# Lagrange-Labs/mapreduce-plonky2

Hardware: AMD Instinct MI355X
Metric: leaf proofs/sec (whole node) + NTT GB/s vs HBM peak, 2^20-row table build, 1/2/4/8 GPU (higher is better)
Workload: dtype u64 (Goldilocks field)

## Files before the change

include/mp2g.h:

```cpp
#ifndef MP2G_H
#define MP2G_H
#include <stddef.h>
#include <stdint.h>
#ifdef __cplusplus
extern "C" {
#endif

typedef struct mp2g_ctx mp2g_ctx;
typedef struct mp2g_tree mp2g_tree;
typedef struct mp2g_batch mp2g_batch;

#define MP2G_POSEIDON2 0
#define MP2G_POSEIDON 1

uint64_t mp2g_stat_leaf_permutations(void);
const char* mp2g_last_error(void);
int mp2g_device_count(void);
int mp2g_ctx_create(int device, mp2g_ctx** out);
void mp2g_ctx_destroy(mp2g_ctx* ctx);
int mp2g_ctx_sync(mp2g_ctx* ctx);
int mp2g_ctx_make_current(mp2g_ctx* ctx);
int mp2g_ctx_mem_info(mp2g_ctx* ctx, size_t* free_bytes, size_t* total_bytes);
void* mp2g_ctx_stream(mp2g_ctx* ctx);
int mp2g_ctx_set_stream(mp2g_ctx* ctx, void* stream);
// ... 9 lines not shown
int mp2g_timer_stop(mp2g_ctx* ctx, float* ms);

int mp2g_ntt(mp2g_ctx* ctx, uint64_t* data, uint32_t log_n, uint32_t batch, int inverse,
             uint64_t coset_shift, int bitrev_out);
int mp2g_ntt_dev(mp2g_ctx* ctx, const uint64_t* d_in, uint64_t* d_out, uint32_t log_n, uint32_t batch,
                 int inverse, uint64_t coset_shift, int bitrev_out);
int mp2g_lde_leaves(mp2g_ctx* ctx, const uint64_t* coeffs, uint32_t log_n, uint32_t w, uint32_t rate_bits,
                    uint64_t* leaves);
int mp2g_lde_dev(mp2g_ctx* ctx, const uint64_t* d_coeffs, uint32_t log_n, uint32_t w, uint32_t rate_bits,
                 uint64_t* d_values);

int mp2g_hash_no_pad_batch(mp2g_ctx* ctx, int variant, const uint64_t* in, uint32_t in_len, uint32_t count,
                           uint32_t out_len, uint64_t* out);
int mp2g_hash_no_pad_batch_dev(mp2g_ctx* ctx, int variant, const uint64_t* d_in, uint32_t in_len,
                               uint32_t count, uint32_t out_len, uint64_t* d_out);
int mp2g_merkle_build(mp2g_ctx* ctx, int variant, const uint64_t* leaves, uint32_t leaf_len,
                      uint32_t log_leaves, uint32_t cap_height, mp2g_tree** out);
int mp2g_merkle_cap(const mp2g_tree* tree, uint64_t* cap );
int mp2g_merkle_open(const mp2g_tree* tree, const uint32_t* idx, uint32_t n_idx, uint64_t* leaves_out,
                     uint64_t* siblings_out);
void mp2g_merkle_free(mp2g_tree* tree);

int mp2g_commit_from_values(mp2g_ctx* ctx, int variant, const uint64_t* values, uint32_t log_n, uint32_t w,
                            uint32_t rate_bits, uint32_t cap_height, mp2g_batch** out);
int mp2g_commit_from_values_dev(mp2g_ctx* ctx, int variant, const uint64_t* d_values, uint32_t log_n,
                                uint32_t w, uint32_t rate_bits, uint32_t cap_height, mp2g_batch** out);
int mp2g_commit_from_coeffs_dev(mp2g_ctx* ctx, int variant, const uint64_t* d_coeffs, uint32_t log_n,
                                uint32_t w, uint32_t rate_bits, uint32_t cap_height, mp2g_batch** out);
int mp2g_recommit_from_values_dev(mp2g_ctx* ctx, mp2g_batch* batch, const uint64_t* d_values);
int mp2g_batch_rehash_dev(mp2g_ctx* ctx, mp2g_batch* batch, int parts);
// ... 21 lines not shown
uint32_t mp2g_reduction_arity_bits(uint32_t degree_bits, uint32_t rate_bits, uint32_t cap_height,
                                   uint32_t arity_bits, uint32_t final_poly_bits, uint32_t* out);
size_t mp2g_fri_proof_words(const mp2g_fri_params* p);
size_t mp2g_fri_n_openings(const mp2g_fri_params* p);

typedef struct mp2g_challenger mp2g_challenger;
int mp2g_challenger_create(mp2g_ctx* ctx, int variant, uint32_t count, mp2g_challenger** out);
int mp2g_challenger_observe(mp2g_challenger* ch, const uint64_t* elems, uint32_t n);
int mp2g_challenger_get(mp2g_challenger* ch, uint32_t n, uint64_t* out );
void mp2g_challenger_free(mp2g_challenger* ch);

int mp2g_fri_fold(mp2g_ctx* ctx, const uint64_t* evals, uint32_t log_m, uint32_t arity_bits,
                  const uint64_t beta[2], uint64_t shift, uint64_t* out);
int mp2g_fri_pow(mp2g_ctx* ctx, int variant, const uint64_t state[12], uint32_t pos, uint32_t bits,
                 uint64_t* witness);

int mp2g_batch_eval_ext(const mp2g_batch* batch, const uint64_t point[2], uint64_t* out );
int mp2g_fri_prove(mp2g_ctx* ctx, const mp2g_fri_params* params, mp2g_batch* const* oracles, const uint64_t zeta[2],
                   mp2g_challenger* ch, uint64_t* proof);

typedef struct mp2g_prover mp2g_prover;
int mp2g_prover_create(mp2g_ctx* ctx, const mp2g_fri_params* params, uint32_t batch, mp2g_prover** out);
int mp2g_prover_set_preprocessed_dev(mp2g_prover* pr, const uint64_t* d_values);
int mp2g_prover_prove_dev(mp2g_prover* pr, const uint64_t* const* d_values, const uint64_t* d_circuit_digest,
                          const uint64_t* d_pi_hash, uint64_t* d_caps, uint64_t* d_openings, uint64_t* d_proof);
void mp2g_prover_free(mp2g_prover* pr);
int mp2g_pcs_prove(mp2g_ctx* ctx, const mp2g_fri_params* params, const uint64_t* const* values,
                   const uint64_t circuit_digest[4], const uint64_t pi_hash[4], uint64_t* caps,
                   uint64_t* openings, uint64_t* proof);

// ... 236 lines not shown
```

mapreduce-plonky2_amd/__init__.py:

```python
import ctypes
import time
import os
import weakref

import numpy as np

_HERE = os.path.dirname(os.path.abspath(__file__))
LIB_PATH = os.environ.get("MP2G_LIB", os.path.join(_HERE, "libmp2gpu.so"))
HEADER_PATH = os.path.join(os.path.dirname(_HERE), "include", "mp2g.h")

P = 0xFFFFFFFF00000001
MULT_GEN = 14293326489335486720
POSEIDON2, POSEIDON = 0, 1

_u64p = ctypes.POINTER(ctypes.c_uint64)
_u32p = ctypes.POINTER(ctypes.c_uint32)
_lib = None


class Mp2gError(RuntimeError):
    pass


def load():
# ... 161 lines not shown
        _ck(load().mp2g_lde_leaves(self.h, _p(c), log_n, w, rate_bits, _p(out)))
        return out

    def lde_dev(self, d_coeffs, log_n, w, rate_bits, d_values):
        _ck(load().mp2g_lde_dev(self.h, d_coeffs.ptr, log_n, w, rate_bits, d_values.ptr))

    def hash_no_pad_batch(self, inputs, out_len=4, variant=POSEIDON2):
        a = _arr(inputs)
        count, in_len = a.shape
        out = np.empty((count, out_len), dtype=np.uint64)
        _ck(load().mp2g_hash_no_pad_batch(self.h, variant, _p(a), in_len, count, out_len, _p(out)))
        return out

    def hash_no_pad(self, values, variant=POSEIDON2):
        return self.hash_no_pad_batch(_arr(values).reshape(1, -1), 4, variant)[0]


class MerkleTree:

    def __init__(self, ctx, leaves, cap_height, variant=POSEIDON2):
        a = _arr(leaves)
        L, leaf_len = a.shape
        self.log_leaves = int(L).bit_length() - 1
        assert 1 << self.log_leaves == L
        self.ctx, self.cap_height, self.leaf_len = ctx, cap_height, leaf_len
        self.h = ctypes.c_void_p()
        _ck(load().mp2g_merkle_build(ctx.h, variant, _p(a), leaf_len, self.log_leaves, cap_height, ctypes.byref(self.h)))
        ctx._adopt(self)

    @property
# ... 160 lines not shown
def fri_fold(ctx, evals, arity_bits, beta, shift):
    a = _arr(evals)
    m = a.shape[0]
    log_m = int(m).bit_length() - 1
    out = np.empty((m >> arity_bits, 2), dtype=np.uint64)
    b = _arr(beta)
    _ck(load().mp2g_fri_fold(ctx.h, _p(a), log_m, arity_bits, _p(b), ctypes.c_uint64(shift), _p(out)))
    return out


def fri_pow(ctx, state, pos, bits, variant=POSEIDON2):
    s = _arr(state)
    w = ctypes.c_uint64()
    _ck(load().mp2g_fri_pow(ctx.h, variant, _p(s), pos, bits, ctypes.byref(w)))
    return w.value


def pcs_prove(ctx, fp, values, circuit_digest, pi_hash):
    vals = [_arr(v) for v in values]
    ptrs = (ctypes.c_void_p * len(vals))(*[v.ctypes.data for v in vals])
    caps = np.empty((fp.n_oracles, fp.cap_words), dtype=np.uint64)
    openings = np.empty((fp.n_openings, 2), dtype=np.uint64)
    proof = np.empty(fp.proof_words, dtype=np.uint64)
    cd, ph = _arr(circuit_digest), _arr(pi_hash)
    _ck(load().mp2g_pcs_prove(ctx.h, ctypes.byref(fp), ptrs, _p(cd), _p(ph), _p(caps), _p(openings), _p(proof)))
    return caps, openings, proof


class Gate(ctypes.Structure):
    _fields_ = [("kind", ctypes.c_uint32), ("p0", ctypes.c_uint32), ("p1", ctypes.c_uint32), ("p2", ctypes.c_uint32),
# ... 572 lines not shown
```

mapreduce-plonky2_amd/csrc/api.hip:

```cpp
#include "ctx.h"
#include <cstdlib>
#include <cstdarg>
#include <cstdio>
#include <cstring>
#include <new>

using namespace mp2g;

static thread_local char g_err[512] = "";
int mp2g::fail(const char* fmt, ...) {
  va_list ap;
  va_start(ap, fmt);
  vsnprintf(g_err, sizeof g_err, fmt, ap);
  va_end(ap);
  return 1;
}

extern "C" {

const char* mp2g_last_error(void) { return g_err; }

int mp2g_device_count(void) {
  int n = 0;
  if (hipGetDeviceCount(&n) != hipSuccess) return 0;
// ... 195 lines not shown
  NEED(out_len >= 1, "out_len >= 1");
  CK(hash_no_pad_batch(c->stream, variant, (const u64*)d_in, in_len, count, out_len, (u64*)d_out));
  return 0;
}
int mp2g_hash_no_pad_batch(mp2g_ctx* c, int variant, const uint64_t* in, uint32_t in_len, uint32_t count,
                           uint32_t out_len, uint64_t* out) {
  NEED(c && out, "ctx/out");
  if (count == 0) return 0;
  DevBuf di, dout;
  CK(di.alloc((size_t)count * in_len * sizeof(u64)));
  CK(dout.alloc((size_t)count * out_len * sizeof(u64)));
  if (in_len) CK(hipMemcpyAsync(di.p, in, (size_t)count * in_len * sizeof(u64), hipMemcpyHostToDevice, c->stream));
  int rc = mp2g_hash_no_pad_batch_dev(c, variant, di.p, in_len, count, out_len, dout.p);
  if (rc) return rc;
  CK(hipMemcpyAsync(out, dout.p, (size_t)count * out_len * sizeof(u64), hipMemcpyDeviceToHost, c->stream));
  CK(hipStreamSynchronize(c->stream));
  return 0;
}

int mp2g_merkle_build(mp2g_ctx* c, int variant, const uint64_t* leaves, uint32_t leaf_len, uint32_t log_leaves,
                      uint32_t cap_height, mp2g_tree** out) {
  NEED(c && out && (leaves || leaf_len == 0), "ctx/out/leaves");
  NEED(variant == 0 || variant == 1, "variant");
  NEED(log_leaves <= 28, "log_leaves <= 28");
  NEED(cap_height <= log_leaves, "cap_height <= log2(leaves)");
  mp2g_tree* t = new (std::nothrow) mp2g_tree();
  if (!t) return fail("out of memory");
  t->ctx = c; t->variant = variant; t->leaf_len = leaf_len; t->log_leaves = log_leaves; t->cap_h = cap_height;
  const size_t L = (size_t)1 << log_leaves;
  hipError_t e = t->leaves.alloc(L * leaf_len * sizeof(u64));
// ... 176 lines not shown
```

mapreduce-plonky2_amd/csrc/fri.hip:

```cpp
#include "fri.h"
#include "poseidon_wave.cuh"

namespace mp2g {

template <int V>
__device__ void ch_duplex(ChState& c) {
  for (u32 i = 0; i < c.n_in; i++) c.state[i] = c.in[i];
  c.n_in = 0;
  u64 s[12];
#pragma unroll
  for (int i = 0; i < 12; i++) s[i] = c.state[i];
  perm<V>(s);
#pragma unroll
  for (int i = 0; i < 12; i++) c.state[i] = s[i];
#pragma unroll
  for (int i = 0; i < 8; i++) c.out[i] = s[i];
  c.n_out = 8;
}
template <int V>
__global__ void ch_kernel(ChState* st, u32 B, const u64* obs, u64 obs_bstride, u32 n_obs, u64* out, u64 out_bstride, u32 n_get) {
  u32 b = blockIdx.x * blockDim.x + threadIdx.x;
  if (b >= B) return;
  ChState c = st[b];
  const u64* o = obs + b * obs_bstride;
// ... 293 lines not shown
  for (int i = 0; i < 8; i++)
    if ((u32)i < pos) base[i] = c.in[i];
  const u64 stride = (u64)gridDim.x * blockDim.x;
  for (u64 cand = (u64)blockIdx.x * blockDim.x + threadIdx.x;; cand += stride) {
    if (threadIdx.x == 0) s_best = atomicMin(wit, ~0ull);
    __syncthreads();
    const unsigned long long best = s_best;
    __syncthreads();
    if (cand - threadIdx.x > best) break;
    u64 s[12];
#pragma unroll
    for (int i = 0; i < 12; i++) s[i] = base[i];
#pragma unroll
    for (int i = 0; i < 8; i++)
      if ((u32)i == pos) s[i] = cand;
    perm<V>(s);
    if (cand < GL_P && (bits == 0 || (s[7] >> (64 - bits)) == 0)) atomicMin(wit, (unsigned long long)cand);
  }
}
__global__ void fill_u64_kernel(u64* p, u64 v, u32 n) {
  u32 i = blockIdx.x * blockDim.x + threadIdx.x;
  if (i < n) p[i] = v;
}

__global__ void __launch_bounds__(256) query_kernel(FriShape sh, FriLayers ly, FriProofLayout L, const u64* chal ,
                                                      u64 chal_bstride, u64* proof) {
  const u32 q = blockIdx.x, b = blockIdx.y, t = threadIdx.x;
  const u32 lg = L.lg;
  const u64 N = (u64)1 << lg;
  u64 x = chal[b * chal_bstride + q] % N;
  u64* const qs = proof + b * L.proof_words + L.q_off + q * L.q_words;
// ... 105 lines not shown
```

mapreduce-plonky2_amd/csrc/gates.hip:

```cpp
#include "gates.h"
#include "poseidon.cuh"
#include "coset_constants.h"

namespace mp2g {

u32 gate_num_constraints(const mp2g_gate& g) {
  switch (g.kind) {
    case MP2G_GATE_CONSTANT: return g.p0;
    case MP2G_GATE_PUBLIC_INPUT: return 4;
    case MP2G_GATE_ARITHMETIC: return g.p0;
    case MP2G_GATE_BASE_SUM: return 1 + g.p0;
    case MP2G_GATE_ARITHMETIC_EXT: case MP2G_GATE_MUL_EXT: return 2 * g.p0;
    case MP2G_GATE_POSEIDON2: case MP2G_GATE_POSEIDON: return 1 + 4 + 36 + 22 + 48 + 12;
    case MP2G_GATE_POSEIDON_MDS: return 24;
    case MP2G_GATE_COSET_INTERPOLATION: return 4 + 4 * (((1u << g.p0) - 2) / (g.p1 - 1));
    case MP2G_GATE_U32_ARITHMETIC: return 36 * g.p0;
    case MP2G_GATE_U32_RANGE_CHECK: return 17 * g.p0;
    case MP2G_GATE_U32_SUBTRACTION: return 19 * g.p0;
    case MP2G_GATE_U32_ADD_MANY: return 21 * g.p1;
    case MP2G_GATE_COMPARISON: return g.p1 ? 6 + 5 * g.p1 + (g.p0 + g.p1 - 1) / g.p1 : 0;
    case MP2G_GATE_EXPONENTIATION: return g.p0 + 1;
    case MP2G_GATE_REDUCING: case MP2G_GATE_REDUCING_EXT: return 2 * g.p0;
    case MP2G_GATE_RANDOM_ACCESS: return (g.p0 + 2) * g.p1 + g.p2;
    case MP2G_GATE_U32_INTERLEAVE: return 34 * g.p0;
// ... 219 lines not shown
        u64 lhs = wire(i), rhs = wire(i + 4), delta = wire(25 + i);
        emit(gl_sub(gl_mul(swap, gl_sub(rhs, lhs)), delta));
        s[i] = gl_add(lhs, delta);
        s[i + 4] = gl_sub(rhs, delta);
      }
#pragma unroll
      for (int i = 8; i < 12; i++) s[i] = wire(i);
      p2_external(s);
#pragma unroll 1
      for (int r = 0; r < 4; r++) {
        if (r != 0) {
#pragma unroll
          for (int i = 0; i < 12; i++) {
            u64 in = wire(29 + 12 * (r - 1) + i);
            emit(diff(s[i], c_p2_ext[12 * r + i], in));
            s[i] = p2_sbox(in, 0);
          }
        } else {
#pragma unroll
          for (int i = 0; i < 12; i++) s[i] = p2_sbox(s[i], c_p2_ext[i]);
        }
        p2_external(s);
      }
      u64 nxt = wire(65);
#pragma unroll 1
      for (int r = 0; r < 22; r++) {
        const u64 in = nxt;
        if (r < 21) nxt = wire(65 + r + 1);
        emit(diff(s[0], c_p2_int[r], in));
        s[0] = p2_sbox(in, 0);
        p2_internal(s);
      }
#pragma unroll 1
      for (int r = 0; r < 4; r++) {
#pragma unroll
        for (int i = 0; i < 12; i++) {
          u64 in = wire(87 + 12 * r + i);
          emit(diff(s[i], c_p2_ext[12 * (4 + r) + i], in));
          s[i] = p2_sbox(in, 0);
        }
        p2_external(s);
      }
#pragma unroll
      for (int i = 0; i < 12; i++) emit(diff0(s[i], wire(12 + i)));
      break;
    }
    case MP2G_GATE_POSEIDON: {
      const u64 swap = wire(24);
      emit(gl_mul(swap, gl_sub(swap, 1)));
      u64 s[12];
#pragma unroll
      for (int i = 0; i < 4; i++) {
        u64 lhs = wire(i), rhs = wire(i + 4), delta = wire(25 + i);
        emit(gl_sub(gl_mul(swap, gl_sub(rhs, lhs)), delta));
        s[i] = gl_add(lhs, delta);
        s[i + 4] = gl_sub(rhs, delta);
      }
#pragma unroll
      for (int i = 8; i < 12; i++) s[i] = wire(i);
#pragma unroll 1
      for (int r = 0; r < 30; r++) {
        if (r >= 4 && r < 26) {
          u64 in = wire(65 + (r - 4));
          emit(diff(s[0], c_p_rc[12 * r], in));
          s[0] = p2_sbox(in, 0);
#pragma unroll
          for (int i = 1; i < 12; i++) s[i] = gl_addw(s[i], c_p_rc[12 * r + i]);
        } else if (r == 0) {
#pragma unroll
          for (int i = 0; i < 12; i++) s[i] = p2_sbox(s[i], c_p_rc[i]);
        } else {
          const int base = r < 4 ? 29 + 12 * (r - 1) : 87 + 12 * (r - 26);
#pragma unroll
          for (int i = 0; i < 12; i++) {
            u64 in = wire(base + i);
            emit(diff(s[i], c_p_rc[12 * r + i], in));
            s[i] = p2_sbox(in, 0);
          }
        }
        poseidon_mds(s);
      }
#pragma unroll
      for (int i = 0; i < 12; i++) emit(diff0(s[i], wire(12 + i)));
      break;
    }
    case MP2G_GATE_POSEIDON_MDS: {
      u64 s0[12], s1[12];
#pragma unroll
      for (int i = 0; i < 12; i++) { s0[i] = wire(2 * i); s1[i] = wire(2 * i + 1); }
      poseidon_mds(s0);
      poseidon_mds(s1);
#pragma unroll
// ... 543 lines not shown
```

mapreduce-plonky2_amd/csrc/merkle.hip:

```cpp
#include "merkle.h"
#include <atomic>
#include "poseidon_wave.cuh"

namespace mp2g {

template <int V>
__global__ void __launch_bounds__(256) leaf_hash_poly_major_kernel(const u64* __restrict__ values, u32 w, u64 stride, u64 n, u64* __restrict__ digests,
                                                                   u64 in_bstride, u64 out_bstride) {
  u64 i = (u64)blockIdx.x * blockDim.x + threadIdx.x;
  if (i >= n) return;
  values += blockIdx.y * in_bstride;
  digests += blockIdx.y * out_bstride;
  u64 s[12];
#pragma unroll
  for (int k = 0; k < 12; k++) s[k] = 0;
  if (w <= 4) {
    for (u32 p = 0; p < w; p++) s[p] = values[p * stride + i];
  } else {
    const u64* v = values + i;
    u32 p = 0;
    for (; p + 8 <= w; p += 8) {
#pragma unroll
      for (int k = 0; k < 8; k++) s[k] = v[(u64)(p + k) * stride];
      perm<V>(s);
    }
    if (p < w) {
#pragma unroll
      for (int k = 0; k < 8; k++)
        if (p + k < w) s[k] = v[(u64)(p + k) * stride];
      perm<V>(s);
    }
  }
  ulonglong2* d = reinterpret_cast<ulonglong2*>(digests + 4 * i);
  d[0] = make_ulonglong2(s[0], s[1]);
  d[1] = make_ulonglong2(s[2], s[3]);
}
template <int V>
__global__ void __launch_bounds__(256) leaf_hash_row_major_kernel(const u64* __restrict__ leaves, u32 len, u64 n, u64* __restrict__ digests) {
  u64 i = (u64)blockIdx.x * blockDim.x + threadIdx.x;
  if (i >= n) return;
  const u64* v = leaves + i * len;
  u64 s[12];
#pragma unroll
  for (int k = 0; k < 12; k++) s[k] = 0;
  if (len <= 4) {
    for (u32 p = 0; p < len; p++) s[p] = v[p];
  } else {
    u32 p = 0;
    for (; p + 8 <= len; p += 8) {
#pragma unroll
      for (int k = 0; k < 8; k++) s[k] = v[p + k];
      perm<V>(s);
    }
    if (p < len) {
#pragma unroll
      for (int k = 0; k < 8; k++)
        if (p + k < len) s[k] = v[p + k];
      perm<V>(s);
    }
  }
#pragma unroll
  for (int k = 0; k < 4; k++) digests[4 * i + k] = s[k];
}
template <int V>
__global__ void __launch_bounds__(256) leaf_hash_ext_soa_kernel(const u64* __restrict__ c0, const u64* __restrict__ c1, u32 arity_bits, u64 n, u64* __restrict__ digests,
                                                                u64 in_bstride, u64 out_bstride) {
  u64 i = (u64)blockIdx.x * blockDim.x + threadIdx.x;
  if (i >= n) return;
  c0 += blockIdx.y * in_bstride;
  c1 += blockIdx.y * in_bstride;
  digests += blockIdx.y * out_bstride;
  u32 arity = 1u << arity_bits;
  const u64* a = c0 + (i << arity_bits);
  const u64* b = c1 + (i << arity_bits);
  u64 s[12];
#pragma unroll
  for (int k = 0; k < 12; k++) s[k] = 0;
  if (arity == 1) {
    s[0] = a[0]; s[1] = b[0];
  } else if (arity == 2) {
    s[0] = a[0]; s[1] = b[0]; s[2] = a[1]; s[3] = b[1];
  } else {
    for (u32 p = 0; p < arity; p += 4) {
#pragma unroll
      for (int k = 0; k < 4; k++) { s[2 * k] = a[p + k]; s[2 * k + 1] = b[p + k]; }
      perm<V>(s);
    }
  }
#pragma unroll
  for (int k = 0; k < 4; k++) digests[4 * i + k] = s[k];
}
template <int V>
__global__ void __launch_bounds__(256) merkle_level_kernel(const u64* __restrict__ in, u64* __restrict__ out, u64 n_out, u64 bstride) {
  u64 i = (u64)blockIdx.x * blockDim.x + threadIdx.x;
  if (i >= n_out) return;
  in += blockIdx.y * bstride;
  out += blockIdx.y * bstride;
  const ulonglong2* src = reinterpret_cast<const ulonglong2*>(in + 8 * i);
  ulonglong2 q0 = src[0], q1 = src[1], q2 = src[2], q3 = src[3];
  u64 s[12] = {q0.x, q0.y, q1.x, q1.y, q2.x, q2.y, q3.x, q3.y, 0, 0, 0, 0};
  perm<V>(s);
  ulonglong2* d = reinterpret_cast<ulonglong2*>(out + 4 * i);
  d[0] = make_ulonglong2(s[0], s[1]);
  d[1] = make_ulonglong2(s[2], s[3]);
}
__global__ void __launch_bounds__(256) merkle_level_wave_kernel(const u64* __restrict__ in, u64* __restrict__ out, u64 n_out, u64 bstride) {
  const u64 gid = (u64)blockIdx.x * blockDim.x + threadIdx.x;
  const u64 iraw = gid >> 4;
  const int l = (int)(gid & 15);
  const bool active = iraw < n_out;
  const u64 i = active ? iraw : n_out - 1;
  in += blockIdx.y * bstride;
  out += blockIdx.y * bstride;
  u64 x = l < 8 ? in[8 * i + l] : 0;
  x = wp2_perm(x, l);
  if (active && l < 4) out[4 * i + l] = x;
}
template <int V>
__global__ void __launch_bounds__(256) hash_no_pad_batch_kernel(const u64* __restrict__ in, u32 in_len, u64 count, u32 out_len, u64* __restrict__ out) {
  u64 i = (u64)blockIdx.x * blockDim.x + threadIdx.x;
  if (i >= count) return;
  const u64* v = in + i * in_len;
  u64 s[12];
#pragma unroll
  for (int k = 0; k < 12; k++) s[k] = 0;
  for (u32 p = 0; p < in_len; p += 8) {
#pragma unroll
    for (int k = 0; k < 8; k++)
      if (p + k < in_len) s[k] = v[p + k];
    perm<V>(s);
  }
  u64* o = out + i * out_len;
  u32 done = 0;
  for (;;) {
#pragma unroll
    for (int k = 0; k < 8; k++) {
      if (done < out_len) o[done] = s[k];
      done++;
    }
    if (done >= out_len) break;
    perm<V>(s);
  }
}
__global__ void merkle_open_kernel(const u64* __restrict__ levels, u32 log_leaves, u32 cap_h, const u32* __restrict__ idx, u32 n_idx, u64* __restrict__ sib) {
  u32 depth = log_leaves - cap_h;
  u32 t = blockIdx.x * blockDim.x + threadIdx.x;
  if (t >= n_idx * depth * 4) return;
  u32 k = t & 3, l = (t >> 2) % depth, q = (t >> 2) / depth;
  u64 off = 0;
  for (u32 j = 0; j < l; j++) off += (u64)4 << (log_leaves - j);
  u32 node = (idx[q] >> l) ^ 1;
  sib[t] = levels[off + 4 * (u64)node + k];
}
__global__ void gather_rows_kernel(const u64* __restrict__ values, u32 w, u64 stride, const u32* __restrict__ idx, u32 n_idx, u64* __restrict__ out) {
  u32 t = blockIdx.x * blockDim.x + threadIdx.x;
  if (t >= n_idx * w) return;
  u32 p = t % w, q = t / w;
// ... 50 lines not shown
  u64* cur = levels;
  if (!batch) return hipSuccess;
  for (u32 lv = log_leaves; lv > cap_h; lv--) {
    u64 n_in = (u64)1 << lv;
    u64* nxt = cur + 4 * n_in;
    if (variant == MP2G_POSEIDON2 && (n_in / 2) * (u64)batch <= 16384) {
      hipLaunchKernelGGL(merkle_level_wave_kernel, grid1(n_in / 2 * 16, 256, batch), dim3(256), 0, st, cur, nxt, n_in / 2, bstride);
    } else
      LAUNCH_V(merkle_level_kernel, grid1(n_in / 2, 256, batch), dim3(256), st, cur, nxt, n_in / 2, bstride);
    cur = nxt;
  }
  return hipGetLastError();
}
hipError_t hash_no_pad_batch(hipStream_t st, int variant, const u64* in, u32 in_len, u64 count, u32 out_len, u64* out) {
  if (!count) return hipSuccess;
  LAUNCH_V(hash_no_pad_batch_kernel, grid1(count, 256), dim3(256), st, in, in_len, count, out_len, out);
  return hipGetLastError();
}
hipError_t merkle_open(hipStream_t st, const u64* levels, u32 log_leaves, u32 cap_h, const u32* idx, u32 n_idx, u64* siblings) {
  u32 total = n_idx * (log_leaves - cap_h) * 4;
  if (!total) return hipSuccess;
  hipLaunchKernelGGL(merkle_open_kernel, grid1(total, 256), dim3(256), 0, st, levels, log_leaves, cap_h, idx, n_idx, siblings);
  return hipGetLastError();
}
hipError_t gather_rows(hipStream_t st, const u64* values, u32 w, u64 stride, const u32* idx, u32 n_idx, u64* out) {
  u32 total = n_idx * w;
  if (!total) return hipSuccess;
  hipLaunchKernelGGL(gather_rows_kernel, grid1(total, 256), dim3(256), 0, st, values, w, stride, idx, n_idx, out);
  return hipGetLastError();
}
hipError_t transpose_to_leaves(hipStream_t st, const u64* values, u32 w, u64 stride, u64 n, u64* out, u32 batch, u64 in_bstride,
// ... 8 lines not shown
```

mapreduce-plonky2_amd/csrc/poseidon.cuh:

```cuda
#pragma once
#include "gl.cuh"
#include "perm_constants.h"

#define MP2G_POSEIDON2 0
#define MP2G_POSEIDON 1

#define c_p2_ext POSEIDON2_RC_EXT
#define c_p2_int POSEIDON2_RC_INT
#define c_p2_diag POSEIDON2_DIAG_M1
#define c_p_rc POSEIDON_RC

GLHD u64 p2_sbox(u64 x, u64 rc) {
  u64 t = gl_addw(x, rc);
  u64 t2 = gl_mulw(t, t), t4 = gl_mulw(t2, t2), t3 = gl_mulw(t, t2);
  return gl_mulw(t3, t4);
}
GLHD void p2_m4_plain(u64& a, u64& b, u64& c, u64& d) {
  u64 t0 = a + b, t1 = c + d;
  u64 t2 = (b << 1) + t1, t3 = (d << 1) + t0;
  u64 t4 = (t1 << 2) + t3, t5 = (t0 << 2) + t2;
  a = t3 + t5; b = t5; c = t2 + t4; d = t4;
}
GLHD void p2_external_half(u64 v[12]) {
  p2_m4_plain(v[0], v[1], v[2], v[3]);
  p2_m4_plain(v[4], v[5], v[6], v[7]);
  p2_m4_plain(v[8], v[9], v[10], v[11]);
#pragma unroll
  for (int i = 0; i < 4; i++) {
    u64 sum = v[i] + v[4 + i] + v[8 + i];
    v[i] += sum; v[4 + i] += sum; v[8 + i] += sum;
  }
}
template <bool RC>
GLHD void p2_external_rc(u64 s[12], const u64* rc) {
  u64 lo[12], hi[12];
#pragma unroll
  for (int i = 0; i < 12; i++) { lo[i] = (u32)s[i]; hi[i] = s[i] >> 32; }
  p2_external_half(lo);
  p2_external_half(hi);
#if defined(__HIP_DEVICE_COMPILE__)
#pragma unroll
  for (int i = 0; i < 12; i++) {
    u64 L = lo[i], H = hi[i];
    if (RC) { L += (u64)(u32)rc[i]; H += rc[i] >> 32; }
    H += L >> 32;
    s[i] = gl_reduce96w(gl_mk((u32)L, (u32)H), H >> 32);
  }
// ... 36 lines not shown
  u64 top = 0;
#pragma unroll
  for (int i = 1; i < 12; i++) {
    bool c = __builtin_add_overflow(acc, s[i], &acc);
    top += c ? 1 : 0;
  }
#pragma unroll
  for (int i = 0; i < 12; i++) {
    u64 lo, hi;
    gl_mul_wide(s[i], c_p2_diag[i], lo, hi);
    bool c = __builtin_add_overflow(lo, acc, &lo);
    s[i] = gl_reduce128w(lo, hi + top + (c ? 1 : 0));
  }
#endif
}
GLHD void poseidon2_perm(u64 s[12]) {
  p2_external_rc<true>(s, c_p2_ext);
#pragma unroll 1
  for (int r = 0; r < 4; r++) {
#pragma unroll
    for (int i = 0; i < 12; i++) s[i] = p2_sbox0(s[i]);
    if (r < 3) p2_external_rc<true>(s, c_p2_ext + 12 * (r + 1)); else p2_external(s);
  }
#pragma unroll 11
  for (int r = 0; r < 22; r++) {
    s[0] = p2_sbox(s[0], c_p2_int[r]);
    p2_internal(s);
  }
#pragma unroll
  for (int i = 0; i < 12; i++) s[i] = gl_addw(s[i], c_p2_ext[48 + i]);
#pragma unroll 1
  for (int r = 4; r < 8; r++) {
#pragma unroll
    for (int i = 0; i < 12; i++) s[i] = p2_sbox0(s[i]);
    if (r < 7) p2_external_rc<true>(s, c_p2_ext + 12 * (r + 1)); else p2_external(s);
  }
#pragma unroll
  for (int i = 0; i < 12; i++) s[i] = gl_canon(s[i]);
}

template <bool RC>
GLHD void poseidon_mds_rc(u64 s[12], const u64* rc) {
  const u32 circ[12] = {17, 15, 41, 16, 2, 28, 13, 13, 39, 18, 34, 20};
  u64 lo[12], hi[12];
#pragma unroll
  for (int i = 0; i < 12; i++) { lo[i] = (u32)s[i]; hi[i] = s[i] >> 32; }
  u64 out[12];
#pragma unroll
  for (int r = 0; r < 12; r++) {
    u64 al = 0, ah = 0;
#pragma unroll
    for (int i = 0; i < 12; i++) {
      al += lo[(i + r) % 12] * circ[i];
// ... 20 lines not shown
#pragma unroll
  for (int i = 0; i < 12; i++) s[i] = gl_addw(s[i], c_p_rc[i]);
#pragma unroll 1
  for (int r = 0; r < 30; r++) {
    if (r < 4 || r >= 26) {
#pragma unroll
      for (int i = 0; i < 12; i++) s[i] = p2_sbox0(s[i]);
    } else {
      s[0] = p2_sbox0(s[0]);
    }
    if (r < 29) poseidon_mds_rc<true>(s, c_p_rc + 12 * (r + 1)); else poseidon_mds(s);
  }
#pragma unroll
  for (int i = 0; i < 12; i++) s[i] = gl_canon(s[i]);
}
template <int VARIANT>
GLHD void perm(u64 s[12]) {
  if (VARIANT == MP2G_POSEIDON2) poseidon2_perm(s); else poseidon_perm(s);
}
template <int VARIANT>
GLD void two_to_one(const u64 l[4], const u64 r[4], u64 out[4]) {
  u64 s[12];
#pragma unroll
  for (int i = 0; i < 4; i++) { s[i] = l[i]; s[4 + i] = r[i]; s[8 + i] = 0; }
  perm<VARIANT>(s);
#pragma unroll
  for (int i = 0; i < 4; i++) out[i] = s[i];
}
```

mapreduce-plonky2_amd/csrc/prover.hip:

```cpp
#include "ctx.h"
#include "fri.h"
#include "zperm.h"
#include "gates.h"
#include "lookup.h"
#include "lookup_wires.h"
#include <cstring>
#include <new>
#include <vector>

using namespace mp2g;


struct mp2g_challenger {
  mp2g_ctx* ctx = nullptr;
  int variant = 0;
  uint32_t count = 0;
  DevBuf st;
};

struct mp2g_prover {
  mp2g_ctx* ctx = nullptr;
  mp2g_fri_params P{};
  uint32_t B = 0;
  uint32_t Bcap = 0;
// ... 155 lines not shown
  std::vector<u64> soa(2 * m);
  for (size_t i = 0; i < m; i++) { soa[i] = evals[2 * i]; soa[m + i] = evals[2 * i + 1]; }
  DevBuf din, dout, db;
  CK(din.alloc(2 * m * sizeof(u64)));
  CK(dout.alloc(2 * m2 * sizeof(u64)));
  CK(db.alloc(2 * sizeof(u64)));
  CK(hipMemcpyAsync(din.p, soa.data(), 2 * m * sizeof(u64), hipMemcpyHostToDevice, c->stream));
  CK(hipMemcpyAsync(db.p, beta, 2 * sizeof(u64), hipMemcpyHostToDevice, c->stream));
  CK(fri_fold_values(c->stream, 1, log_m, arity_bits, din.p, 0, dout.p, 0, db.p, 0, shift));
  std::vector<u64> res(2 * m2);
  CK(hipMemcpyAsync(res.data(), dout.p, 2 * m2 * sizeof(u64), hipMemcpyDeviceToHost, c->stream));
  CK(hipStreamSynchronize(c->stream));
  for (size_t i = 0; i < m2; i++) { out[2 * i] = res[i]; out[2 * i + 1] = res[m2 + i]; }
  return 0;
}
int mp2g_fri_pow(mp2g_ctx* c, int variant, const uint64_t state[12], uint32_t pos, uint32_t bits, uint64_t* witness) {
  NEED(c && state && witness, "ctx/pointers");
  NEED(variant == 0 || variant == 1, "variant");
  NEED(pos < 8 && bits <= 32, "pos < 8, bits <= 32");
  ChState h{};
  for (int i = 0; i < 12; i++) h.state[i] = state[i];
  for (uint32_t i = 0; i < pos; i++) h.in[i] = state[i];
  h.n_in = pos;
  DevBuf ds, dw;
  CK(ds.alloc(sizeof(ChState)));
  CK(dw.alloc(FRI_POW_STRIDE * sizeof(u64)));
  CK(hipMemcpyAsync(ds.p, &h, sizeof h, hipMemcpyHostToDevice, c->stream));
  CK(fri_pow(c->stream, variant, (const ChState*)ds.p, 1, bits, dw.p));
  CK(hipMemcpyAsync(witness, dw.p, sizeof(u64), hipMemcpyDeviceToHost, c->stream));
  CK(hipStreamSynchronize(c->stream));
  return 0;
}

static int prover_create_impl(mp2g_ctx* c, const mp2g_fri_params* params, uint32_t batch, bool alloc_oracles, mp2g_prover** out) {
  NEED(c && out, "ctx/out");
  NEED(batch >= 1 && batch <= 4096, "1 <= batch <= 4096");
  int rc = params_check(params);
  if (rc) return rc;
  mp2g_prover* pr = new (std::nothrow) mp2g_prover();
  if (!pr) return fail("out of memory");
  pr->ctx = c; pr->P = *params; pr->B = pr->Bcap = batch;
  const mp2g_fri_params& P = pr->P;
  const size_t n = (size_t)1 << P.log_n, N = n << P.rate_bits, B = batch;
  const uint32_t lg = P.log_n + P.rate_bits;
  pr->L = fri_proof_layout(P);
  pr->levels_words = merkle_levels_words(lg, P.cap_height);
// ... 606 lines not shown
```

Baseline: 890.6.

## Skip dead final-layer work in Poseidon2 permutations for absorb and digest lanes

Adds a templated Poseidon2 permutation that computes only the live output lanes of the last external layer and can skip canonicalisation. Intermediate absorb steps in leaf hashing and sponge use it, and so do digest-only hashes, two-to-one compression and the FRI proof-of-work search. The aim is to cut ALU work in the hash-heavy leaf and Merkle kernels. It also adds batched leaf-hash, Merkle-level and PoW API entry points, and the gate code switches to a specialised sbox call. The risk is a correctness error if the partial-lane output is not actually dead downstream, for example non-canonical intermediate states.

```diff
diff --git a/include/mp2g.h b/include/mp2g.h
--- a/include/mp2g.h
+++ b/include/mp2g.h
@@ -47,6 +47,12 @@
                            uint32_t out_len, uint64_t* out);
 int mp2g_hash_no_pad_batch_dev(mp2g_ctx* ctx, int variant, const uint64_t* d_in, uint32_t in_len,
                                uint32_t count, uint32_t out_len, uint64_t* d_out);
+int mp2g_leaf_hash_batch(mp2g_ctx* ctx, int variant, const uint64_t* values, uint32_t w, uint32_t n, uint32_t batch,
+                         uint64_t* digests);
+int mp2g_leaf_hash_ext_batch(mp2g_ctx* ctx, int variant, const uint64_t* values, uint32_t arity_bits, uint32_t n,
+                             uint32_t batch, uint64_t* digests);
+int mp2g_merkle_levels_batch(mp2g_ctx* ctx, int variant, const uint64_t* digests, uint32_t log_leaves,
+                             uint32_t cap_height, uint32_t batch, uint64_t* levels);
 int mp2g_merkle_build(mp2g_ctx* ctx, int variant, const uint64_t* leaves, uint32_t leaf_len,
                       uint32_t log_leaves, uint32_t cap_height, mp2g_tree** out);
 int mp2g_merkle_cap(const mp2g_tree* tree, uint64_t* cap );
@@ -98,6 +104,8 @@
                   const uint64_t beta[2], uint64_t shift, uint64_t* out);
 int mp2g_fri_pow(mp2g_ctx* ctx, int variant, const uint64_t state[12], uint32_t pos, uint32_t bits,
                  uint64_t* witness);
+int mp2g_fri_pow_batch(mp2g_ctx* ctx, int variant, const uint64_t* states, uint32_t count, uint32_t pos, uint32_t bits,
+                       uint64_t* witnesses);
 
 int mp2g_batch_eval_ext(const mp2g_batch* batch, const uint64_t point[2], uint64_t* out );
 int mp2g_fri_prove(mp2g_ctx* ctx, const mp2g_fri_params* params, mp2g_batch* const* oracles, const uint64_t zeta[2],
diff --git a/mapreduce-plonky2_amd/__init__.py b/mapreduce-plonky2_amd/__init__.py
--- a/mapreduce-plonky2_amd/__init__.py
+++ b/mapreduce-plonky2_amd/__init__.py
@@ -199,6 +199,28 @@
 
     def hash_no_pad(self, values, variant=POSEIDON2):
         return self.hash_no_pad_batch(_arr(values).reshape(1, -1), 4, variant)[0]
+
+    def leaf_hash_batch(self, values, variant=POSEIDON2):
+        a = _arr(values)
+        batch, w, n = a.shape
+        out = np.empty((batch, n, 4), dtype=np.uint64)
+        _ck(load().mp2g_leaf_hash_batch(self.h, variant, _p(a), w, n, batch, _p(out)))
+        return out
+
+    def leaf_hash_ext_batch(self, values, arity_bits, variant=POSEIDON2):
+        a = _arr(values)
+        batch, n = a.shape[0], a.shape[2] >> arity_bits
+        out = np.empty((batch, n, 4), dtype=np.uint64)
+        _ck(load().mp2g_leaf_hash_ext_batch(self.h, variant, _p(a), arity_bits, n, batch, _p(out)))
+        return out
+
+    def merkle_levels_batch(self, digests, cap_height, variant=POSEIDON2):
+        a = _arr(digests)
+        batch, n = a.shape[0], a.shape[1]
+        log_leaves = int(n).bit_length() - 1
+        out = np.empty((batch, 4 * (2 * n - (1 << cap_height))), dtype=np.uint64)
+        _ck(load().mp2g_merkle_levels_batch(self.h, variant, _p(a), log_leaves, cap_height, batch, _p(out)))
+        return out
 
 
 class MerkleTree:
@@ -389,6 +411,13 @@
     w = ctypes.c_uint64()
     _ck(load().mp2g_fri_pow(ctx.h, variant, _p(s), pos, bits, ctypes.byref(w)))
     return w.value
+
+
+def fri_pow_batch(ctx, states, pos, bits, variant=POSEIDON2):
+    s = _arr(states)
+    out = np.empty(s.shape[0], dtype=np.uint64)
+    _ck(load().mp2g_fri_pow_batch(ctx.h, variant, _p(s), s.shape[0], pos, bits, _p(out)))
+    return out
 
 
 def pcs_prove(ctx, fp, values, circuit_digest, pi_hash):
diff --git a/mapreduce-plonky2_amd/csrc/api.hip b/mapreduce-plonky2_amd/csrc/api.hip
--- a/mapreduce-plonky2_amd/csrc/api.hip
+++ b/mapreduce-plonky2_amd/csrc/api.hip
@@ -233,6 +233,51 @@
   int rc = mp2g_hash_no_pad_batch_dev(c, variant, di.p, in_len, count, out_len, dout.p);
   if (rc) return rc;
   CK(hipMemcpyAsync(out, dout.p, (size_t)count * out_len * sizeof(u64), hipMemcpyDeviceToHost, c->stream));
+  CK(hipStreamSynchronize(c->stream));
+  return 0;
+}
+
+int mp2g_leaf_hash_batch(mp2g_ctx* c, int variant, const uint64_t* values, uint32_t w, uint32_t n, uint32_t batch, uint64_t* digests) {
+  NEED(c && digests && (values || !w), "ctx/pointers");
+  NEED(variant == 0 || variant == 1, "variant");
+  if (!n || !batch) return 0;
+  const size_t in_words = (size_t)batch * w * n, out_words = (size_t)batch * n * 4;
+  DevBuf di, dout;
+  CK(di.alloc((in_words ? in_words : 1) * sizeof(u64)));
+  CK(dout.alloc(out_words * sizeof(u64)));
+  if (in_words) CK(hipMemcpyAsync(di.p, values, in_words * sizeof(u64), hipMemcpyHostToDevice, c->stream));
+  CK(leaf_hash_poly_major(c->stream, variant, di.p, w, n, n, dout.p, batch, (u64)w * n, (u64)n * 4));
+  CK(hipMemcpyAsync(digests, dout.p, out_words * sizeof(u64), hipMemcpyDeviceToHost, c->stream));
+  CK(hipStreamSynchronize(c->stream));
+  return 0;
+}
+int mp2g_leaf_hash_ext_batch(mp2g_ctx* c, int variant, const uint64_t* values, uint32_t arity_bits, uint32_t n, uint32_t batch, uint64_t* digests) {
+  NEED(c && values && digests, "ctx/pointers");
+  NEED(variant == 0 || variant == 1, "variant");
+  NEED(arity_bits >= 1 && arity_bits <= 4, "1 <= arity_bits <= 4");
+  if (!n || !batch) return 0;
+  const size_t m = (size_t)n << arity_bits, in_words = (size_t)batch * 2 * m, out_words = (size_t)batch * n * 4;
+  DevBuf di, dout;
+  CK(di.alloc(in_words * sizeof(u64)));
+  CK(dout.alloc(out_words * sizeof(u64)));
+  CK(hipMemcpyAsync(di.p, values, in_words * sizeof(u64), hipMemcpyHostToDevice, c->stream));
+  CK(leaf_hash_ext_soa(c->stream, variant, di.p, di.p + m, arity_bits, n, dout.p, batch, 2 * m, (u64)n * 4));
+  CK(hipMemcpyAsync(digests, dout.p, out_words * sizeof(u64), hipMemcpyDeviceToHost, c->stream));
+  CK(hipStreamSynchronize(c->stream));
+  return 0;
+}
+int mp2g_merkle_levels_batch(mp2g_ctx* c, int variant, const uint64_t* digests, uint32_t log_leaves, uint32_t cap_height, uint32_t batch,
+                             uint64_t* levels) {
+  NEED(c && digests && levels, "ctx/pointers");
+  NEED(variant == 0 || variant == 1, "variant");
+  NEED(log_leaves <= 28 && cap_height <= log_leaves, "cap_height <= log_leaves <= 28");
+  if (!batch) return 0;
+  const size_t lw = merkle_levels_words(log_leaves, cap_height), leaf_words = (size_t)4 << log_leaves;
+  DevBuf dl;
+  CK(dl.alloc(batch * lw * sizeof(u64)));
+  CK(hipMemcpy2DAsync(dl.p, lw * sizeof(u64), digests, leaf_words * sizeof(u64), leaf_words * sizeof(u64), batch, hipMemcpyHostToDevice, c->stream));
+  CK(merkle_reduce(c->stream, variant, dl.p, log_leaves, cap_height, batch, lw));
+  CK(hipMemcpyAsync(levels, dl.p, batch * lw * sizeof(u64), hipMemcpyDeviceToHost, c->stream));
   CK(hipStreamSynchronize(c->stream));
   return 0;
 }
diff --git a/mapreduce-plonky2_amd/csrc/fri.hip b/mapreduce-plonky2_amd/csrc/fri.hip
--- a/mapreduce-plonky2_amd/csrc/fri.hip
+++ b/mapreduce-plonky2_amd/csrc/fri.hip
@@ -331,7 +331,7 @@
 #pragma unroll
     for (int i = 0; i < 8; i++)
       if ((u32)i == pos) s[i] = cand;
-    perm<V>(s);
+    perm<V, 7, 8, true>(s);
     if (cand < GL_P && (bits == 0 || (s[7] >> (64 - bits)) == 0)) atomicMin(wit, (unsigned long long)cand);
   }
 }
diff --git a/mapreduce-plonky2_amd/csrc/gates.hip b/mapreduce-plonky2_amd/csrc/gates.hip
--- a/mapreduce-plonky2_amd/csrc/gates.hip
+++ b/mapreduce-plonky2_amd/csrc/gates.hip
@@ -257,7 +257,7 @@
           for (int i = 0; i < 12; i++) {
             u64 in = wire(29 + 12 * (r - 1) + i);
             emit(diff(s[i], c_p2_ext[12 * r + i], in));
-            s[i] = p2_sbox(in, 0);
+            s[i] = p2_sbox0(in);
           }
         } else {
 #pragma unroll
@@ -271,7 +271,7 @@
         const u64 in = nxt;
         if (r < 21) nxt = wire(65 + r + 1);
         emit(diff(s[0], c_p2_int[r], in));
-        s[0] = p2_sbox(in, 0);
+        s[0] = p2_sbox0(in);
         p2_internal(s);
       }
 #pragma unroll 1
@@ -280,7 +280,7 @@
         for (int i = 0; i < 12; i++) {
           u64 in = wire(87 + 12 * r + i);
           emit(diff(s[i], c_p2_ext[12 * (4 + r) + i], in));
-          s[i] = p2_sbox(in, 0);
+          s[i] = p2_sbox0(in);
         }
         p2_external(s);
       }
@@ -306,7 +306,7 @@
         if (r >= 4 && r < 26) {
           u64 in = wire(65 + (r - 4));
           emit(diff(s[0], c_p_rc[12 * r], in));
-          s[0] = p2_sbox(in, 0);
+          s[0] = p2_sbox0(in);
 #pragma unroll
           for (int i = 1; i < 12; i++) s[i] = gl_addw(s[i], c_p_rc[12 * r + i]);
         } else if (r == 0) {
@@ -318,7 +318,7 @@
           for (int i = 0; i < 12; i++) {
             u64 in = wire(base + i);
             emit(diff(s[i], c_p_rc[12 * r + i], in));
-            s[i] = p2_sbox(in, 0);
+            s[i] = p2_sbox0(in);
           }
         }
         poseidon_mds(s);
diff --git a/mapreduce-plonky2_amd/csrc/merkle.hip b/mapreduce-plonky2_amd/csrc/merkle.hip
--- a/mapreduce-plonky2_amd/csrc/merkle.hip
+++ b/mapreduce-plonky2_amd/csrc/merkle.hip
@@ -19,17 +19,19 @@
   } else {
     const u64* v = values + i;
     u32 p = 0;
-    for (; p + 8 <= w; p += 8) {
+    for (; p + 16 <= w; p += 8) {
 #pragma unroll
       for (int k = 0; k < 8; k++) s[k] = v[(u64)(p + k) * stride];
-      perm<V>(s);
-    }
-    if (p < w) {
+      perm<V, 8, 12, false>(s);
+    }
+    for (; p < w; p += 8) {
 #pragma unroll
       for (int k = 0; k < 8; k++)
         if (p + k < w) s[k] = v[(u64)(p + k) * stride];
-      perm<V>(s);
-    }
+      perm<V, 0, 12, false>(s);
+    }
+#pragma unroll
+    for (int k = 0; k < 4; k++) s[k] = gl_canon(s[k]);
   }
   ulonglong2* d = reinterpret_cast<ulonglong2*>(digests + 4 * i);
   d[0] = make_ulonglong2(s[0], s[1]);
@@ -47,17 +49,19 @@
     for (u32 p = 0; p < len; p++) s[p] = v[p];
   } else {
     u32 p = 0;
-    for (; p + 8 <= len; p += 8) {
+    for (; p + 16 <= len; p += 8) {
 #pragma unroll
       for (int k = 0; k < 8; k++) s[k] = v[p + k];
-      perm<V>(s);
-    }
-    if (p < len) {
+      perm<V, 8, 12, false>(s);
+    }
+    for (; p < len; p += 8) {
 #pragma unroll
       for (int k = 0; k < 8; k++)
         if (p + k < len) s[k] = v[p + k];
-      perm<V>(s);
-    }
+      perm<V, 0, 12, false>(s);
+    }
+#pragma unroll
+    for (int k = 0; k < 4; k++) s[k] = gl_canon(s[k]);
   }
 #pragma unroll
   for (int k = 0; k < 4; k++) digests[4 * i + k] = s[k];
@@ -81,11 +85,15 @@
   } else if (arity == 2) {
     s[0] = a[0]; s[1] = b[0]; s[2] = a[1]; s[3] = b[1];
   } else {
-    for (u32 p = 0; p < arity; p += 4) {
+    u32 p = 0;
+    for (; p + 4 < arity; p += 4) {
 #pragma unroll
       for (int k = 0; k < 4; k++) { s[2 * k] = a[p + k]; s[2 * k + 1] = b[p + k]; }
-      perm<V>(s);
-    }
+      perm<V, 8, 12, false>(s);
+    }
+#pragma unroll
+    for (int k = 0; k < 4; k++) { s[2 * k] = a[p + k]; s[2 * k + 1] = b[p + k]; }
+    perm<V, 0, 4, true>(s);
   }
 #pragma unroll
   for (int k = 0; k < 4; k++) digests[4 * i + k] = s[k];
@@ -99,7 +107,7 @@
   const ulonglong2* src = reinterpret_cast<const ulonglong2*>(in + 8 * i);
   ulonglong2 q0 = src[0], q1 = src[1], q2 = src[2], q3 = src[3];
   u64 s[12] = {q0.x, q0.y, q1.x, q1.y, q2.x, q2.y, q3.x, q3.y, 0, 0, 0, 0};
-  perm<V>(s);
+  perm<V, 0, 4, true>(s);
   ulonglong2* d = reinterpret_cast<ulonglong2*>(out + 4 * i);
   d[0] = make_ulonglong2(s[0], s[1]);
   d[1] = make_ulonglong2(s[2], s[3]);
@@ -116,19 +124,31 @@
   x = wp2_perm(x, l);
   if (active && l < 4) out[4 * i + l] = x;
 }
-template <int V>
-__global__ void __launch_bounds__(256) hash_no_pad_batch_kernel(const u64* __restrict__ in, u32 in_len, u64 count, u32 out_len, u64* __restrict__ out) {
+template <int V, bool NARROW>
+GLD void hash_no_pad_lane(const u64* __restrict__ in, u32 in_len, u64 count, u32 out_len, u64* __restrict__ out) {
   u64 i = (u64)blockIdx.x * blockDim.x + threadIdx.x;
   if (i >= count) return;
   const u64* v = in + i * in_len;
   u64 s[12];
 #pragma unroll
   for (int k = 0; k < 12; k++) s[k] = 0;
-  for (u32 p = 0; p < in_len; p += 8) {
+  u32 p = 0;
+  for (; p + 16 <= in_len; p += 8) {
+#pragma unroll
+    for (int k = 0; k < 8; k++) s[k] = v[p + k];
+    perm<V, 8, 12, false>(s);
+  }
+  if (p + 8 < in_len) {
+#pragma unroll
+    for (int k = 0; k < 8; k++) s[k] = v[p + k];
+    perm<V, 0, 12, false>(s);
+    p += 8;
+  }
+  if (p < in_len) {
 #pragma unroll
     for (int k = 0; k < 8; k++)
       if (p + k < in_len) s[k] = v[p + k];
-    perm<V>(s);
+    perm<V, 0, NARROW ? 4 : 12, true>(s);
   }
   u64* o = out + i * out_len;
   u32 done = 0;
@@ -138,9 +158,17 @@
       if (done < out_len) o[done] = s[k];
       done++;
     }
-    if (done >= out_len) break;
+    if (NARROW || done >= out_len) break;
     perm<V>(s);
   }
+}
+template <int V>
+__global__ void __launch_bounds__(256) hash_no_pad_batch_kernel(const u64* __restrict__ in, u32 in_len, u64 count, u32 out_len, u64* __restrict__ out) {
+  hash_no_pad_lane<V, false>(in, in_len, count, out_len, out);
+}
+template <int V>
+__global__ void __launch_bounds__(256) hash_no_pad_digest_kernel(const u64* __restrict__ in, u32 in_len, u64 count, u32 out_len, u64* __restrict__ out) {
+  hash_no_pad_lane<V, true>(in, in_len, count, out_len, out);
 }
 __global__ void merkle_open_kernel(const u64* __restrict__ levels, u32 log_leaves, u32 cap_h, const u32* __restrict__ idx, u32 n_idx, u64* __restrict__ sib) {
   u32 depth = log_leaves - cap_h;
@@ -221,7 +249,8 @@
 }
 hipError_t hash_no_pad_batch(hipStream_t st, int variant, const u64* in, u32 in_len, u64 count, u32 out_len, u64* out) {
   if (!count) return hipSuccess;
-  LAUNCH_V(hash_no_pad_batch_kernel, grid1(count, 256), dim3(256), st, in, in_len, count, out_len, out);
+  if (out_len <= 4) LAUNCH_V(hash_no_pad_digest_kernel, grid1(count, 256), dim3(256), st, in, in_len, count, out_len, out);
+  else LAUNCH_V(hash_no_pad_batch_kernel, grid1(count, 256), dim3(256), st, in, in_len, count, out_len, out);
   return hipGetLastError();
 }
 hipError_t merkle_open(hipStream_t st, const u64* levels, u32 log_leaves, u32 cap_h, const u32* idx, u32 n_idx, u64* siblings) {
diff --git a/mapreduce-plonky2_amd/csrc/poseidon.cuh b/mapreduce-plonky2_amd/csrc/poseidon.cuh
--- a/mapreduce-plonky2_amd/csrc/poseidon.cuh
+++ b/mapreduce-plonky2_amd/csrc/poseidon.cuh
@@ -21,16 +21,22 @@
   u64 t4 = (t1 << 2) + t3, t5 = (t0 << 2) + t2;
   a = t3 + t5; b = t5; c = t2 + t4; d = t4;
 }
-GLHD void p2_external_half(u64 v[12]) {
+template <int LO, int HI>
+GLHD void p2_external_half_live(u64 v[12]) {
   p2_m4_plain(v[0], v[1], v[2], v[3]);
   p2_m4_plain(v[4], v[5], v[6], v[7]);
   p2_m4_plain(v[8], v[9], v[10], v[11]);
 #pragma unroll
   for (int i = 0; i < 4; i++) {
+    const bool l0 = i >= LO && i < HI, l1 = 4 + i >= LO && 4 + i < HI, l2 = 8 + i >= LO && 8 + i < HI;
+    if (!(l0 || l1 || l2)) continue;
     u64 sum = v[i] + v[4 + i] + v[8 + i];
-    v[i] += sum; v[4 + i] += sum; v[8 + i] += sum;
-  }
-}
+    if (l0) v[i] += sum;
+    if (l1) v[4 + i] += sum;
+    if (l2) v[8 + i] += sum;
+  }
+}
+GLHD void p2_external_half(u64 v[12]) { p2_external_half_live<0, 12>(v); }
 template <bool RC>
 GLHD void p2_external_rc(u64 s[12], const u64* rc) {
   u64 lo[12], hi[12];
@@ -97,7 +103,7 @@
   }
 #endif
 }
-GLHD void poseidon2_perm(u64 s[12]) {
+GLHD void p2_perm_front(u64 s[12]) {
   p2_external_rc<true>(s, c_p2_ext);
 #pragma unroll 1
   for (int r = 0; r < 4; r++) {
@@ -112,6 +118,9 @@
   }
 #pragma unroll
   for (int i = 0; i < 12; i++) s[i] = gl_addw(s[i], c_p2_ext[48 + i]);
+}
+GLHD void poseidon2_perm(u64 s[12]) {
+  p2_perm_front(s);
 #pragma unroll 1
   for (int r = 4; r < 8; r++) {
 #pragma unroll
@@ -120,6 +129,33 @@
   }
 #pragma unroll
   for (int i = 0; i < 12; i++) s[i] = gl_canon(s[i]);
+}
+template <int LO, int HI, bool CANON>
+GLHD void poseidon2_perm_live(u64 s[12]) {
+#if defined(__HIP_DEVICE_COMPILE__)
+  p2_perm_front(s);
+#pragma unroll 1
+  for (int r = 4;; r++) {
+#pragma unroll
+    for (int i = 0; i < 12; i++) s[i] = p2_sbox0(s[i]);
+    if (r == 7) break;
+    p2_external_rc<true>(s, c_p2_ext + 12 * (r + 1));
+  }
+  u64 lo[12], hi[12];
+#pragma unroll
+  for (int i = 0; i < 12; i++) { lo[i] = (u32)s[i]; hi[i] = s[i] >> 32; }
+  p2_external_half_live<LO, HI>(lo);
+  p2_external_half_live<LO, HI>(hi);
+#pragma unroll
+  for (int i = LO; i < HI; i++) {
+    u64 L = lo[i], H = hi[i];
+    H += L >> 32;
+    s[i] = gl_reduce96w(gl_mk((u32)L, (u32)H), H >> 32);
+    if (CANON) s[i] = gl_canon(s[i]);
+  }
+#else
+  poseidon2_perm(s);
+#endif
 }
 
 template <bool RC>
@@ -170,9 +206,11 @@
 #pragma unroll
   for (int i = 0; i < 12; i++) s[i] = gl_canon(s[i]);
 }
-template <int VARIANT>
+template <int VARIANT, int LO = 0, int HI = 12, bool CANON = true>
 GLHD void perm(u64 s[12]) {
-  if (VARIANT == MP2G_POSEIDON2) poseidon2_perm(s); else poseidon_perm(s);
+  if (VARIANT != MP2G_POSEIDON2) poseidon_perm(s);
+  else if (LO == 0 && HI == 12 && CANON) poseidon2_perm(s);
+  else poseidon2_perm_live<LO, HI, CANON>(s);
 }
 template <int VARIANT>
 GLD void two_to_one(const u64 l[4], const u64 r[4], u64 out[4]) {
diff --git a/mapreduce-plonky2_amd/csrc/prover.hip b/mapreduce-plonky2_amd/csrc/prover.hip
--- a/mapreduce-plonky2_amd/csrc/prover.hip
+++ b/mapreduce-plonky2_amd/csrc/prover.hip
@@ -193,22 +193,31 @@
   for (size_t i = 0; i < m2; i++) { out[2 * i] = res[i]; out[2 * i + 1] = res[m2 + i]; }
   return 0;
 }
-int mp2g_fri_pow(mp2g_ctx* c, int variant, const uint64_t state[12], uint32_t pos, uint32_t bits, uint64_t* witness) {
-  NEED(c && state && witness, "ctx/pointers");
+int mp2g_fri_pow_batch(mp2g_ctx* c, int variant, const uint64_t* states, uint32_t count, uint32_t pos, uint32_t bits, uint64_t* witnesses) {
+  NEED(c && states && witnesses, "ctx/pointers");
   NEED(variant == 0 || variant == 1, "variant");
   NEED(pos < 8 && bits <= 32, "pos < 8, bits <= 32");
-  ChState h{};
-  for (int i = 0; i < 12; i++) h.state[i] = state[i];
-  for (uint32_t i = 0; i < pos; i++) h.in[i] = state[i];
-  h.n_in = pos;
+  NEED(count >= 1 && count <= 4096, "1 <= count <= 4096");
+  std::vector<ChState> h(count);
+  for (uint32_t b = 0; b < count; b++) {
+    h[b] = ChState{};
+    for (int i = 0; i < 12; i++) h[b].state[i] = states[12 * b + i];
+    for (uint32_t i = 0; i < pos; i++) h[b].in[i] = states[12 * b + i];
+    h[b].n_in = pos;
+  }
+  std::vector<u64> w((size_t)count * FRI_POW_STRIDE);
   DevBuf ds, dw;
-  CK(ds.alloc(sizeof(ChState)));
-  CK(dw.alloc(FRI_POW_STRIDE * sizeof(u64)));
-  CK(hipMemcpyAsync(ds.p, &h, sizeof h, hipMemcpyHostToDevice, c->stream));
-  CK(fri_pow(c->stream, variant, (const ChState*)ds.p, 1, bits, dw.p));
-  CK(hipMemcpyAsync(witness, dw.p, sizeof(u64), hipMemcpyDeviceToHost, c->stream));
+  CK(ds.alloc(count * sizeof(ChState)));
+  CK(dw.alloc(w.size() * sizeof(u64)));
+  CK(hipMemcpyAsync(ds.p, h.data(), count * sizeof(ChState), hipMemcpyHostToDevice, c->stream));
+  CK(fri_pow(c->stream, variant, (const ChState*)ds.p, count, bits, dw.p));
+  CK(hipMemcpyAsync(w.data(), dw.p, w.size() * sizeof(u64), hipMemcpyDeviceToHost, c->stream));
   CK(hipStreamSynchronize(c->stream));
-  return 0;
+  for (uint32_t b = 0; b < count; b++) witnesses[b] = w[(size_t)b * FRI_POW_STRIDE];
+  return 0;
+}
+int mp2g_fri_pow(mp2g_ctx* c, int variant, const uint64_t state[12], uint32_t pos, uint32_t bits, uint64_t* witness) {
+  return mp2g_fri_pow_batch(c, variant, state, 1, pos, bits, witness);
 }
 
 static int prover_create_impl(mp2g_ctx* c, const mp2g_fri_params* params, uint32_t batch, bool alloc_oracles, mp2g_prover** out) {
```

After: 893.2 (median of 6 runs). No clear change (+0.3%).
